# galacticglum/composer

Hardware: AMD Instinct MI355X
Metric: MIDI-event tokens/sec (train, seq=1024) (higher is better)
Workload: dtype bf16; 1 GPU; 6L/8H/d512 Transformer train step, seq=1024, B=128/GPU, dropout 0.10, Adam lr 1e-3, synthetic int32 event ids (vocab 390), random-init weights; global_batch=128, seq_len=1024, parallelism=dp1

## Files before the change

### composer_amd/csrc/attention.hip

```cpp
#include "common.h"

typedef __attribute__((address_space(3))) bf16x4 lds_bf16x4;

__device__ __forceinline__ int rho(int r, int h) { return (r & 3) + 8 * (r >> 2) + 4 * h; }
__device__ __forceinline__ void both_halves(float v, float& a, float& b) {
    uint32_t u = __builtin_bit_cast(uint32_t, v), u2 = u;
    asm volatile("s_nop 1\n\tv_permlane32_swap_b32 %0, %1" : "+v"(u), "+v"(u2));
    const uint32_t r[2] = {u, u2};
    a = __builtin_bit_cast(float, r[0]);
    b = __builtin_bit_cast(float, r[1]);
}
__device__ __forceinline__ float half_max(float v) { float a, b; both_halves(v, a, b); return fmaxf(a, b); }
__device__ __forceinline__ float half_sum(float v) { float a, b; both_halves(v, a, b); return a + b; }

template <typename T> struct AT;
template <> struct AT<bf16_t> {
    static constexpr int KSTEP = 16;
    static constexpr int VN = 8;
    typedef bf16x8 frag;
    static constexpr bool EXACT = false;
};
template <> struct AT<float> {
    static constexpr int KSTEP = 2;
    static constexpr int VN = 4;
    typedef float frag;
    static constexpr bool EXACT = true;
};

template <typename T> using frag_t = typename AT<T>::frag;

template <typename T, int D> struct Occ {
    static constexpr int MINW = (std::is_same<T, float>::value && D == 128) ? 1 : 2;
#ifndef ATTN_MINW_Q
#define ATTN_MINW_Q 3
#endif
    static constexpr int MINW_Q = (std::is_same<T, bf16_t>::value && D <= 64) ? ATTN_MINW_Q : MINW;
};

template <typename T, int D> struct Geo {
    static constexpr int DP = D < 32 ? 32 : D;
    static constexpr int DT = DP / 32;
    static constexpr int S = std::is_same<T, float>::value ? DP + 1 : DP + 8;
    static constexpr int NS = D / AT<T>::KSTEP;
};

template <typename T> __device__ __forceinline__ f32x16 mfma32(frag_t<T> a, frag_t<T> b, f32x16 c);
template <> __device__ __forceinline__ f32x16 mfma32<bf16_t>(bf16x8 a, bf16x8 b, f32x16 c) {
    return __builtin_amdgcn_mfma_f32_32x32x16_bf16(a, b, c, 0, 0, 0);
}
template <> __device__ __forceinline__ f32x16 mfma32<float>(float a, float b, f32x16 c) {
    return __builtin_amdgcn_mfma_f32_32x32x2f32(a, b, c, 0, 0, 0);
}

template <typename T, int D>
__device__ __forceinline__ void stage_rows(T* img, const T* __restrict__ g, int64_t gstride, int row0, int row_end,
                                           int nrows, int tid) {
    constexpr int VN = AT<T>::VN, DP = Geo<T, D>::DP, S = Geo<T, D>::S;
    constexpr int CPR = DP / VN;
    for (int c = tid; c < nrows * CPR; c += 256) {
        int r = c / CPR, cc = c % CPR;
        Vec16<T> v;
#pragma unroll
        for (int j = 0; j < VN; j++) v.set(j, 0.f);
        if (row0 + r < row_end && cc * VN < D) v = ld16(g + (int64_t)(row0 + r) * gstride + cc * VN);
        if (std::is_same<T, float>::value) {
#pragma unroll
            for (int j = 0; j < VN; j++) img[r * S + cc * VN + j] = from_f32<T>(v.get(j));
        } else {
            st16(img + r * S + cc * VN, v);
        }
    }
}

template <typename T, int D, int ROWS = 64> struct Stager {
    static constexpr int VN = AT<T>::VN, DP = Geo<T, D>::DP, S = Geo<T, D>::S;
    static constexpr int CPR = (D < DP ? D : DP) / VN;
    static constexpr int NC = (ROWS * CPR + 255) / 256;
    static constexpr bool WHOLE = (ROWS * CPR) % 256 == 0;
    Vec16<T> r[NC];
    __device__ __forceinline__ void load(const T* __restrict__ g, int64_t gstride, int row0, int row_end, int tid) {
        if constexpr (!std::is_same<T, float>::value || D >= 32) {
            typedef __attribute__((ext_vector_type(4))) uint32_t u32x4;
            const int64_t span = ((int64_t)(row_end - 1) * gstride + D) * (int64_t)sizeof(T);
            const __amdgpu_buffer_rsrc_t rsrc = __builtin_amdgcn_make_buffer_rsrc((void*)g, 0, (int)span, 0x00020000);
#pragma unroll
            for (int i = 0; i < NC; i++) {
                const int c = tid + 256 * i;
                const int row = c / CPR, cc = c % CPR;
                int off = (int)(((int64_t)(row0 + row) * gstride + cc * VN) * (int64_t)sizeof(T));
                if (!WHOLE && c >= ROWS * CPR) off = 0x7FFFFFF0;
                const u32x4 w = __builtin_amdgcn_raw_buffer_load_b128(rsrc, off, 0, 0);
                r[i].v = __builtin_bit_cast(decltype(r[i].v), w);
            }
            return;
        }
#pragma unroll
        for (int i = 0; i < NC; i++) {
            const int c = tid + 256 * i;
            const int row = c / CPR, cc = c % CPR;
#pragma unroll
            for (int j = 0; j < VN; j++) r[i].set(j, 0.f);
            if (c < ROWS * CPR && row0 + row < row_end && cc * VN < D) r[i] = ld16(g + (int64_t)(row0 + row) * gstride + cc * VN);
        }
    }
    __device__ __forceinline__ void store(T* img, int tid) const {
#pragma unroll
        for (int i = 0; i < NC; i++) {
            const int c = tid + 256 * i;
            const int row = c / CPR, cc = c % CPR;
            if (WHOLE || c < ROWS * CPR) {
                if constexpr (std::is_same<T, float>::value) {
#pragma unroll
                    for (int j = 0; j < VN; j++) img[row * S + cc * VN + j] = r[i].get(j);
                } else {
                    st16(img + row * S + cc * VN, r[i]);
                }
            }
        }
    }
};

template <typename T, int D>
__device__ __forceinline__ void load_bfrags(frag_t<T>* f, const T* __restrict__ g,
                                            int64_t gstride, int row, bool valid, int h) {
    constexpr int NS = Geo<T, D>::NS;
#pragma unroll
    for (int s = 0; s < NS; s++) {
        if constexpr (std::is_same<T, float>::value) {
            f[s] = valid ? g[(int64_t)row * gstride + 2 * s + h] : 0.f;
        } else {
            bf16x8 z;
#pragma unroll
            for (int j = 0; j < 8; j++) z[j] = (bf16_t)0.f;
            f[s] = valid ? *reinterpret_cast<const bf16x8*>(g + (int64_t)row * gstride + 16 * s + 8 * h) : z;
        }
    }
}

template <typename T, int D>
__device__ __forceinline__ f32x16 mma_rows(const T* img, int row0, const frag_t<T>* bf,
                                           int lane, f32x16 acc) {
    constexpr int NS = Geo<T, D>::NS, S = Geo<T, D>::S;
    const int r = row0 + (lane & 31), h = lane >> 5;
#pragma unroll
    for (int s = 0; s < NS; s++) {
        frag_t<T> a;
        if constexpr (std::is_same<T, float>::value) a = img[r * S + 2 * s + h];
        else a = *reinterpret_cast<const bf16x8*>(img + r * S + 16 * s + 8 * h);
        acc = mfma32<T>(a, bf[s], acc);
    }
    return acc;
}

template <typename T, int D>
__device__ __forceinline__ f32x16 mma_acc_b(const T* img, int krow0, int dt, const f32x16& x, int lane, f32x16 acc) {
    constexpr int S = Geo<T, D>::S;
    const int h = lane >> 5;
    if constexpr (std::is_same<T, float>::value) {
#pragma unroll
        for (int r = 0; r < 16; r++) {
            float a = img[(krow0 + rho(r, h)) * S + 32 * dt + (lane & 31)];
            acc = __builtin_amdgcn_mfma_f32_32x32x2f32(a, x[r], acc, 0, 0, 0);
        }
    } else {
        const int G = lane >> 4, q = (lane & 15) >> 2, p = lane & 3;
        const int col = 32 * dt + 16 * (G & 1) + 4 * p;
#pragma unroll
        for (int s = 0; s < 2; s++) {
            const int kr = krow0 + 16 * s + 4 * (G >> 1) + q;
            bf16x4 lo = __builtin_amdgcn_ds_read_tr16_b64_v4bf16((lds_bf16x4*)(img + kr * S + col));
            bf16x4 hi = __builtin_amdgcn_ds_read_tr16_b64_v4bf16((lds_bf16x4*)(img + (kr + 8) * S + col));
            bf16x8 a, b;
#pragma unroll
            for (int j = 0; j < 4; j++) {
                a[j] = lo[j];
                a[4 + j] = hi[j];
            }
#pragma unroll
            for (int j = 0; j < 8; j++) b[j] = (bf16_t)x[8 * s + j];
            acc = __builtin_amdgcn_mfma_f32_32x32x16_bf16(a, b, acc, 0, 0, 0);
        }
    }
    return acc;
}

#define LOG2E_F 1.4426950408889634f
__device__ __forceinline__ float fast_exp2(float x) { return __builtin_amdgcn_exp2f(x); }
__device__ __forceinline__ float max3(float a, float b, float c) { return fmaxf(fmaxf(a, b), c); }
__device__ __forceinline__ float max16(const f32x16& s) {
    float a = max3(s[0], s[1], s[2]), b = max3(s[3], s[4], s[5]), c = max3(s[6], s[7], s[8]);
    float d = max3(s[9], s[10], s[11]), e = max3(s[12], s[13], s[14]);
    return max3(max3(a, b, c), max3(d, e, s[15]), a);
}

__device__ __forceinline__ f32x2 exp2_scaled16(f32x16& s, float c, float negm, f32x2 sum) {
    float s0 = sum[0], s1 = sum[1];
#pragma unroll
    for (int r = 0; r < 16; r += 2) {
        const float p0 = fast_exp2(fmaf(s[r], c, negm)), p1 = fast_exp2(fmaf(s[r + 1], c, negm));
        s0 += p0;
        s1 += p1;
        s[r] = p0;
        s[r + 1] = p1;
    }
    return f32x2{s0, s1};
}
__device__ __forceinline__ void pin16(f32x16& v) {
#pragma unroll
    for (int r = 0; r < 16; r++) {
        float x = v[r];
        asm("" : "+v"(x));
        v[r] = x;
    }
}

template <bool PIN = false>
__device__ __forceinline__ void mask16_qlane(f32x16& v, uint32_t rowh, int k0, int h, uint32_t thr) {
    const uint32_t gg = ((uint32_t)(k0 >> 2) + (uint32_t)h) * ATTN_G;
#pragma unroll
    for (int g4 = 0; g4 < 4; g4++) {
        const uint32_t x = rowh ^ (gg + (uint32_t)(2 * g4) * ATTN_G);
        v[4 * g4 + 0] = (__umul24(x, ATTN_C0) >= thr) ? v[4 * g4 + 0] : 0.f;
        v[4 * g4 + 1] = (__umul24(x, ATTN_C1) >= thr) ? v[4 * g4 + 1] : 0.f;
        v[4 * g4 + 2] = (__umul24(x, ATTN_C2) >= thr) ? v[4 * g4 + 2] : 0.f;
        v[4 * g4 + 3] = (__umul24(x, ATTN_C3) >= thr) ? v[4 * g4 + 3] : 0.f;
    }
    if (PIN) pin16(v);
}

template <typename T, int D>
__device__ __forceinline__ void store_t_tile(T* __restrict__ out, int64_t ostride, int row, bool valid, int dt,
                                             const f32x16& y, float mul, int h) {
    if constexpr (std::is_same<T, bf16_t>::value && D % 32 == 0) {
#pragma unroll
        for (int gp = 0; gp < 4; gp += 2) {
            uint32_t w[2][2];
#pragma unroll
            for (int k = 0; k < 2; k++)
#pragma unroll
                for (int j = 0; j < 2; j++) {
                    typedef __attribute__((ext_vector_type(2))) __bf16 bf2;
                    const bf2 t = {(bf16_t)(y[4 * (gp + k) + 2 * j] * mul), (bf16_t)(y[4 * (gp + k) + 2 * j + 1] * mul)};
                    w[k][j] = __builtin_bit_cast(uint32_t, t);
                }
#pragma unroll
            for (int j = 0; j < 2; j++) asm volatile("s_nop 1\n\tv_permlane32_swap_b32 %0, %1" : "+v"(w[0][j]), "+v"(w[1][j]));
            typedef __attribute__((ext_vector_type(4))) uint32_t u32x4;
            const u32x4 v = {w[0][0], w[0][1], w[1][0], w[1][1]};
            if (valid) *reinterpret_cast<u32x4*>(out + (int64_t)row * ostride + 32 * dt + 8 * (gp + h)) = v;
        }
        return;
    }
    if (!valid) return;
#pragma unroll
    for (int g = 0; g < 4; g++) {
        int d = 32 * dt + 8 * g + 4 * h;
        if (d < D) {
            if constexpr (std::is_same<T, float>::value) {
                f32x4 v = {y[4 * g] * mul, y[4 * g + 1] * mul, y[4 * g + 2] * mul, y[4 * g + 3] * mul};
                *reinterpret_cast<f32x4*>(out + (int64_t)row * ostride + d) = v;
            } else {
                bf16x4 v;
#pragma unroll
                for (int j = 0; j < 4; j++) v[j] = (bf16_t)(y[4 * g + j] * mul);
                *reinterpret_cast<bf16x4*>(out + (int64_t)row * ostride + d) = v;
            }
        }
    }
}

template <typename T, int D>
__device__ __forceinline__ void colsum_t_tiles(float* __restrict__ bias_grad, bool valid, const f32x16* y, float mul, int h,
                                               int lane) {
    constexpr int DT = Geo<T, D>::DT;
    const int l = lane & 31;
#pragma unroll
    for (int t0 = 0; t0 < DT; t0 += 2) {
        constexpr int dummy = 0;
        (void)dummy;
        const bool pair = t0 + 1 < DT;
        float v[32];
#pragma unroll
        for (int r = 0; r < 16; r++) {
            v[r] = valid ? y[t0][r] * mul : 0.f;
            v[16 + r] = (pair && valid) ? y[pair ? t0 + 1 : t0][r] * mul : 0.f;
        }
        if (pair) {
#pragma unroll
            for (int k = 0; k < 16; k++) {
                const float keep = (l & 16) ? v[k + 16] : v[k], send = (l & 16) ? v[k] : v[k + 16];
                v[k] = keep + __shfl_xor(send, 16);
            }
        } else {
#pragma unroll
            for (int k = 0; k < 16; k++) v[k] += __shfl_xor(v[k], 16);
        }
#pragma unroll
        for (int s = 8; s >= 1; s >>= 1) {
#pragma unroll
            for (int k = 0; k < s; k++) {
                const float keep = (l & s) ? v[k + s] : v[k], send = (l & s) ? v[k] : v[k + s];
                v[k] = keep + __shfl_xor(send, s);
            }
        }
        const int idx = pair ? l : (l & 15);
        const int d = 32 * (t0 + (idx >> 4)) + 8 * ((idx & 15) >> 2) + 4 * h + (idx & 3);
        if ((pair || l < 16) && d < D) atomicAdd(bias_grad + d, v[0]);
    }
}

__device__ __forceinline__ int pair_block(int ph, int nb, int x) {
    if ((int)gridDim.x == nb && nb > 1) return ph == 0 ? nb - 1 - x : -1;
    const int hi = nb - 1 - x;
    if (ph == 0) return hi;
    return x < hi ? x : -1;
}

__device__ __forceinline__ void xcd_block(int& bx, int& by, int H) {
    const int gx = gridDim.x, gy = gridDim.y;
    if (gy & 7) { bx = blockIdx.x; by = blockIdx.y; return; }
    const int L = blockIdx.x + gx * blockIdx.y;
    const int xcd = L & 7, slot = L >> 3;
    bx = slot % gx;
    by = (slot / gx) * 8 + xcd;
    const int bb = by / H;
    by = bb * H + (by % H + bb) % H;
}

__device__ __forceinline__ void attn_job(int plan_u, int nb, int H, int& by, int& qb0, int& qb1) {
    if (plan_u < 0) {
// ... 532 lines not shown
            const bool more = qts + QT < Tn;
            const int qt0 = qts + wq;
            if (more) {
                sq.load(qg, rs, qts + QT, Tn, tid);
                so.load(dog, E, qts + QT, Tn, tid);
                load_rows(qts + QT);
            }
#pragma unroll
            for (int sub = 0; sub < 2; sub++) {
                const int qb0 = qt0 + 32 * sub;
                if (!INT && (qb0 + 31 < k0w || qb0 >= Tn || k0w >= Tn)) continue;
                f32x16 s, dp;
#pragma unroll
                for (int r = 0; r < 16; r++) { s[r] = 0.f; dp[r] = 0.f; }
                s = mma_rows<T, D>(Qs, 32 * sub, kf, lane, s);
                dp = mma_rows<T, D>(Os, 32 * sub, vf, lane, dp);
                f32x4 lq[4], dq4[4];
                __attribute__((ext_vector_type(4))) uint32_t rh4[4];
#pragma unroll
                for (int g = 0; g < 4; g++) {
                    const int ql = 32 * sub + 8 * g + 4 * h;
                    lq[g] = *reinterpret_cast<const f32x4*>(Ls + ql);
                    dq4[g] = *reinterpret_cast<const f32x4*>(Ls + QT + ql);
                    if constexpr (DROP) rh4[g] = *reinterpret_cast<const __attribute__((ext_vector_type(4))) uint32_t*>(Ls + 2 * QT + ql);
                }
                f32x16 pt;
#pragma unroll
                for (int r = 0; r < 16; r++) {
                    if constexpr (EXACT) pt[r] = expf(s[r] * scale - lq[r >> 2][r & 3]);
                    else pt[r] = fast_exp2(fmaf(s[r], c2, -lq[r >> 2][r & 3]));
                }
                if constexpr (!INT) {
                    const bool edge = EXACT || (qb0 < k0w + 32) || (qb0 + 32 > Tn) || (k0w + 32 > Tn);
                    if (edge) {
#pragma unroll
                        for (int r = 0; r < 16; r++) {
                            const int qq = qt0 + 32 * sub + rho(r, h);
                            if ((key > qq) || (qq >= Tn) || !kvalid) pt[r] = 0.f;
                        }
                    }
                }
#pragma unroll
                for (int r = 0; r < 16; r++) {
                    const float p = pt[r];
                    if constexpr (EXACT || !DROP) {
                        float dpv = dp[r];
                        float pd = p;
                        if constexpr (DROP) {
                            const bool keep = __umul24(rh4[r >> 2][r & 3] ^ kgG, kC) >= drop.thr;
                            dpv = keep ? dpv : 0.f;
                            pd = keep ? p : 0.f;
                        }
                        pt[r] = pd;
                        s[r] = p * (dpv - dq4[r >> 2][r & 3]);
                    } else {
                        const bool keep = __umul24(rh4[r >> 2][r & 3] ^ kgG, kC) >= drop.thr;
                        const float pd = keep ? p : 0.f;
                        pt[r] = pd;
                        s[r] = fmaf(pd, dp[r], -(p * dq4[r >> 2][r & 3]));
                    }
                }
#pragma unroll
                for (int dt = 0; dt < G::DT; dt++) {
                    dv[dt] = mma_acc_b<T, D>(Os, 32 * sub, dt, pt, lane, dv[dt]);
                    dk[dt] = mma_acc_b<T, D>(Qs, 32 * sub, dt, s, lane, dk[dt]);
                }
            }
            if (more) {
                if constexpr (KS) __syncthreads();
                T* nbuf = Qb + (KS ? 0 : (sb ^ 1)) * 2 * IMG;
                sq.store(nbuf, tid);
                so.store(nbuf + IMG, tid);
                store_rows(Lb + (KS ? 0 : (sb ^ 1)) * 3 * QT, qts + QT);
            }
            __syncthreads();
        };
        int qt0 = qstart, it = 0;
        const int diag_end = EXACT ? Tn : min(Tn, KS ? k0w + 32 : qstart + 128);
        for (; qt0 < diag_end; qt0 += QT, it++) tile(std::false_type{}, qt0, it);
        for (; qt0 + QT <= Tn; qt0 += QT, it++) tile(std::true_type{}, qt0, it);
        for (; qt0 < Tn; qt0 += QT, it++) tile(std::false_type{}, qt0, it);
        if constexpr (KS) {
            float* mg = reinterpret_cast<float*>(smem_raw);
            if (wave > 0) {
#pragma unroll
                for (int dt = 0; dt < G::DT; dt++)
#pragma unroll
                    for (int r = 0; r < 16; r++) {
                        mg[(((wave - 1) * 2 * G::DT + 2 * dt) * 16 + r) * 64 + lane] = dk[dt][r];
                        mg[(((wave - 1) * 2 * G::DT + 2 * dt + 1) * 16 + r) * 64 + lane] = dv[dt][r];
                    }
            }
            __syncthreads();
            if (wave > 0) continue;
#pragma unroll
            for (int w = 0; w < 3; w++)
#pragma unroll
                for (int dt = 0; dt < G::DT; dt++)
#pragma unroll
                    for (int r = 0; r < 16; r++) {
                        dk[dt][r] += mg[((w * 2 * G::DT + 2 * dt) * 16 + r) * 64 + lane];
                        dv[dt][r] += mg[((w * 2 * G::DT + 2 * dt + 1) * 16 + r) * 64 + lane];
                    }
        }
        const float row_rs = (lr.rstd && kvalid) ? lr.rstd[(int64_t)b * Tn + key] : 1.f;
#pragma unroll
        for (int dt = 0; dt < G::DT; dt++) {
            store_t_tile<T, D>(dkg, rs, key, kvalid, dt, dk[dt], scale * keep_scale * row_rs, h);
            store_t_tile<T, D>(dvg, rs, key, kvalid, dt, dv[dt], keep_scale * row_rs, h);
        }
        if (bias_grad) {
            colsum_t_tiles<T, D>(bias_grad + E + hd * D, kvalid, dk, scale * keep_scale, h, lane);
            colsum_t_tiles<T, D>(bias_grad + 2 * E + hd * D, kvalid, dv, keep_scale, h, lane);
        }
    }
}
template <typename T, int D, bool DROP>
__global__ __launch_bounds__(256, (Occ<T, D>::MINW)) void attn_dkv_kernel(const T* __restrict__ qkv, const T* __restrict__ d_o,
                                                                          const float* __restrict__ lse,
                                                                          const float* __restrict__ delta, T* __restrict__ dqkv,
                                                                          float* __restrict__ bias_grad, int Tn, int H, float scale,
                                                                          DropCfg drop) {
    attn_dkv_body<T, D, DROP, 0>(qkv, d_o, lse, delta, dqkv, bias_grad, Tn, H, scale, drop, nullptr, 0);
}
template <typename T, int D, bool DROP>
__global__ __launch_bounds__(256, (Occ<T, D>::MINW)) void attn_dkv_ln_kernel(const T* __restrict__ qkv, const T* __restrict__ d_o,
                                                                          const float* __restrict__ lse,
                                                                          const float* __restrict__ delta, T* __restrict__ dqkv,
                                                                          float* __restrict__ bias_grad, int Tn, int H, float scale,
                                                                          DropCfg drop, AttnLnRows lr) {
    attn_dkv_body<T, D, DROP, 0>(qkv, d_o, lse, delta, dqkv, bias_grad, Tn, H, scale, drop, nullptr, 0, lr);
}
template <typename T, int D, bool DROP>
__global__ __launch_bounds__(256, 2) void attn_bwd_ks_kernel(const T* __restrict__ qkv, const T* __restrict__ o, const T* __restrict__ d_o,
                                                             const float* __restrict__ lse, float* __restrict__ delta, T* __restrict__ dqkv,
                                                             float* __restrict__ bias_grad, int Tn, int H, float scale, DropCfg drop) {
    const int x = blockIdx.x, nqb = (int)gridDim.x >> 1;
    if (x & 1) attn_dq_body<T, D, DROP, 1>(qkv, o, d_o, lse, delta, dqkv, bias_grad, Tn, H, scale, drop, -1, nqb - 1 - (x >> 1));
    else attn_dkv_body<T, D, DROP, 2>(qkv, d_o, lse, delta, dqkv, bias_grad, Tn, H, scale, drop, o, x >> 1);
}
template <typename T, int D, bool DROP>
__global__ __launch_bounds__(256, 2) void attn_dq_ks_kernel(const T* __restrict__ qkv, const T* __restrict__ o, const T* __restrict__ d_o,
                                                            const float* __restrict__ lse, float* __restrict__ delta, T* __restrict__ dqkv,
                                                            float* __restrict__ bias_grad, int Tn, int H, float scale, DropCfg drop) {
    attn_dq_body<T, D, DROP, 1>(qkv, o, d_o, lse, delta, dqkv, bias_grad, Tn, H, scale, drop, -1, (int)gridDim.x - 1 - (int)blockIdx.x);
}
template <typename T, int D, bool DROP>
__global__ __launch_bounds__(256, 2) void attn_dkv_ks_kernel(const T* __restrict__ qkv, const T* __restrict__ d_o, const float* __restrict__ lse,
                                                             const float* __restrict__ delta, T* __restrict__ dqkv, float* __restrict__ bias_grad,
                                                             int Tn, int H, float scale, DropCfg drop) {
    attn_dkv_body<T, D, DROP, 1>(qkv, d_o, lse, delta, dqkv, bias_grad, Tn, H, scale, drop, nullptr, (int)blockIdx.x);
}

int colsum_run(void* stream, const void* X, int ldx, float* out, int rows, int cols, int dtype, float* det_ws, size_t det_ws_bytes);
static int attn_grid_x(int Tn, int BH) {
    const int nb = cdiv(Tn, 128), pairs = (nb + 1) / 2;
    return (nb > 1 && (int64_t)pairs * BH < 512) ? nb : pairs;
}
static int attn_plan_u(int Tn, int BH, int wgs_per_cu) {
    const int nb = cdiv(Tn, 128), pairs = (nb + 1) / 2;
    if (nb < 2 || (BH & 7) || (int64_t)pairs * BH < 512 || wgs_per_cu < 1) return -1;
    const int rows_x = BH / 8, slots = 32 * wgs_per_cu;
    const int rounds = rows_x * pairs / slots;
    const int paired_rows = rounds > 0 ? rounds * slots / pairs : rows_x / 4;
    const int u = rows_x - paired_rows;
    return u > 0 ? u : -1;
}
static dim3 attn_plan_grid(int Tn, int BH, int u) {
    if (u < 0) return dim3(attn_grid_x(Tn, BH), BH);
    const int nb = cdiv(Tn, 128), pairs = (nb + 1) / 2, rows_x = BH / 8;
    return dim3(8 * ((rows_x - u) * pairs + u * nb), 1);
}
static bool attn_key_split(int Tn, int BH, int D, bool bf16) {
    if (!bf16 || D > 32 || Tn < 64) return false;
    static const int mode = [] { const char* e = getenv("COMPOSER_ATTN_KS"); return e ? atoi(e) : -1; }();
    if (mode == 0) return false;
    if (mode == 1) return true;
    return (int64_t)cdiv(Tn, 128) * BH <= 128;
}
template <typename K> static int attn_wgs_per_cu(K kernel, size_t smem) {
    int n = 0;
    if (hipOccupancyMaxActiveBlocksPerMultiprocessor(&n, kernel, 256, smem) != hipSuccess) { (void)hipGetLastError(); return 0; }
    return n;
}
template <typename T, int D> static size_t attn_ks_smem() { return 4 * 256 * Geo<T, D>::S * sizeof(T); }
template <typename T, int D> static bool attn_ks_available() {
    static const bool ok = [] {
        const int ks = (int)attn_ks_smem<T, D>(), kv = ks / 2 + 3 * 256 * (int)sizeof(float);
        const void* big[] = {(const void*)attn_fwd_kernel<T, D, true, false, true>, (const void*)attn_fwd_kernel<T, D, false, false, true>,
                             (const void*)attn_bwd_ks_kernel<T, D, true>, (const void*)attn_bwd_ks_kernel<T, D, false>,
                             (const void*)attn_dq_ks_kernel<T, D, true>, (const void*)attn_dq_ks_kernel<T, D, false>};
        const void* half[] = {(const void*)attn_dkv_ks_kernel<T, D, true>, (const void*)attn_dkv_ks_kernel<T, D, false>};
        bool good = true;
        for (const void* f : big) good = good && hipFuncSetAttribute(f, hipFuncAttributeMaxDynamicSharedMemorySize, ks) == hipSuccess;
        for (const void* f : half) good = good && hipFuncSetAttribute(f, hipFuncAttributeMaxDynamicSharedMemorySize, kv) == hipSuccess;
        if (!good) (void)hipGetLastError();
        return good;
    }();
    return ok;
}
template <typename T, int D>
static int launch_fwd(hipStream_t s, const void* qkv, void* o, float* lse, int B, int Tn, int H, float scale, DropCfg d,
                      const float* amask) {
    if constexpr (std::is_same<T, bf16_t>::value && D <= 32) {
        const size_t smem_ks = attn_ks_smem<T, D>();
        if (!amask && attn_ks_available<T, D>() && attn_key_split(Tn, B * H, D, true)) {
            const dim3 grid(cdiv(Tn, 32), B * H);
            PROF_START(3, s);
            if (d.thr) attn_fwd_kernel<T, D, true, false, true><<<grid, 256, smem_ks, s>>>((const T*)qkv, (T*)o, lse, Tn, H, scale, d, -1, nullptr);
            else attn_fwd_kernel<T, D, false, false, true><<<grid, 256, smem_ks, s>>>((const T*)qkv, (T*)o, lse, Tn, H, scale, d, -1, nullptr);
            PROF_STOP(3, s, 2.0 * B * H * (double)Tn * Tn * D, (double)B * Tn * H * (4.0 * D * sizeof(T) + 4.0));
            KERNEL_CHECK();
            return CMP_OK;
        }
    }
    size_t smem = 4 * 64 * Geo<T, D>::S * sizeof(T);
    if (smem > 65536) {
        HIP_CHECK(hipFuncSetAttribute((const void*)attn_fwd_kernel<T, D, true>, hipFuncAttributeMaxDynamicSharedMemorySize, (int)smem));
        HIP_CHECK(hipFuncSetAttribute((const void*)attn_fwd_kernel<T, D, false>, hipFuncAttributeMaxDynamicSharedMemorySize, (int)smem));
    }
    static const int wgs_per_cu = attn_wgs_per_cu(attn_fwd_kernel<T, D, true>, smem);
    const int plan_u = attn_plan_u(Tn, B * H, wgs_per_cu);
    const dim3 grid = attn_plan_grid(Tn, B * H, plan_u);
    const double flops = 2.0 * B * H * (double)Tn * Tn * D;
    if (amask) {
        if (smem > 65536) {
            HIP_CHECK(hipFuncSetAttribute((const void*)attn_fwd_kernel<T, D, true, true>, hipFuncAttributeMaxDynamicSharedMemorySize, (int)smem));
            HIP_CHECK(hipFuncSetAttribute((const void*)attn_fwd_kernel<T, D, false, true>, hipFuncAttributeMaxDynamicSharedMemorySize, (int)smem));
        }
        if (d.thr) attn_fwd_kernel<T, D, true, true><<<grid, 256, smem, s>>>((const T*)qkv, (T*)o, lse, Tn, H, scale, d, plan_u, amask);
        else attn_fwd_kernel<T, D, false, true><<<grid, 256, smem, s>>>((const T*)qkv, (T*)o, lse, Tn, H, scale, d, plan_u, amask);
        KERNEL_CHECK();
        return CMP_OK;
    }
    PROF_START(3, s);
    if (d.thr) attn_fwd_kernel<T, D, true><<<grid, 256, smem, s>>>((const T*)qkv, (T*)o, lse, Tn, H, scale, d, plan_u, nullptr);
    else attn_fwd_kernel<T, D, false><<<grid, 256, smem, s>>>((const T*)qkv, (T*)o, lse, Tn, H, scale, d, plan_u, nullptr);
    PROF_STOP(3, s, flops, (double)B * Tn * H * (4.0 * D * sizeof(T) + 4.0));
    KERNEL_CHECK();
    return CMP_OK;
}
template <typename T, int D>
static int launch_bwd(hipStream_t s, const void* qkv, const void* o, const void* d_o, const float* lse, float* delta,
                      void* dqkv, int B, int Tn, int H, float scale, DropCfg d, float* bias_grad, AttnLnRows lr) {
    if constexpr (std::is_same<T, bf16_t>::value) {
        if (lr.rstd) {
            size_t smem = 4 * 64 * Geo<T, D>::S * sizeof(T);
            if (smem + 1536 > 65536) {
                HIP_CHECK(hipFuncSetAttribute((const void*)attn_dq_ln_kernel<T, D, true>, hipFuncAttributeMaxDynamicSharedMemorySize, (int)smem));
                HIP_CHECK(hipFuncSetAttribute((const void*)attn_dq_ln_kernel<T, D, false>, hipFuncAttributeMaxDynamicSharedMemorySize, (int)smem));
                HIP_CHECK(hipFuncSetAttribute((const void*)attn_dkv_ln_kernel<T, D, true>, hipFuncAttributeMaxDynamicSharedMemorySize, (int)smem + 1536));
                HIP_CHECK(hipFuncSetAttribute((const void*)attn_dkv_ln_kernel<T, D, false>, hipFuncAttributeMaxDynamicSharedMemorySize, (int)smem + 1536));
            }
            const double fl = (double)B * H * (double)Tn * Tn * D;
            static const int wgs_per_cu_ln = attn_wgs_per_cu(attn_dq_ln_kernel<T, D, true>, smem);
            const int plan_u = attn_plan_u(Tn, B * H, wgs_per_cu_ln);
            const dim3 qgrid = attn_plan_grid(Tn, B * H, plan_u);
            const dim3 kgrid(attn_grid_x(Tn, B * H), B * H);
            PROF_START(4, s);
            if (d.thr) attn_dq_ln_kernel<T, D, true><<<qgrid, 256, smem, s>>>((const T*)qkv, (const T*)o, (const T*)d_o, lse, delta, (T*)dqkv, bias_grad, Tn, H, scale, d, plan_u, lr);
            else attn_dq_ln_kernel<T, D, false><<<qgrid, 256, smem, s>>>((const T*)qkv, (const T*)o, (const T*)d_o, lse, delta, (T*)dqkv, bias_grad, Tn, H, scale, d, plan_u, lr);
            PROF_STOP(4, s, 3.0 * fl, (double)B * Tn * H * (6.0 * D * sizeof(T) + 8.0));
            KERNEL_CHECK();
            PROF_START(5, s);
            if (d.thr) attn_dkv_ln_kernel<T, D, true><<<kgrid, 256, smem + 384 * sizeof(float), s>>>((const T*)qkv, (const T*)d_o, lse, delta, (T*)dqkv, bias_grad, Tn, H, scale, d, lr);
            else attn_dkv_ln_kernel<T, D, false><<<kgrid, 256, smem + 384 * sizeof(float), s>>>((const T*)qkv, (const T*)d_o, lse, delta, (T*)dqkv, bias_grad, Tn, H, scale, d, lr);
            PROF_STOP(5, s, 4.0 * fl, (double)B * Tn * H * (6.0 * D * sizeof(T) + 8.0));
            KERNEL_CHECK();
            return CMP_OK;
        }
    } else {
        CMP_REQUIRE(!lr.rstd, "attention backward: LayerNorm row scaling exists in bf16 only");
    }
    if constexpr (std::is_same<T, bf16_t>::value && D <= 32) {
        const size_t smem_ks = attn_ks_smem<T, D>(), smem_kv = smem_ks / 2 + 3 * 256 * sizeof(float);
        if (attn_ks_available<T, D>() && attn_key_split(Tn, B * H, D, true)) {
            const double flk = (double)B * H * (double)Tn * Tn * D;
            float* const bias_out = bias_grad;
            bias_grad = nullptr;
            auto bias_pass = [&]() -> int {
                return bias_out ? colsum_run(s, dqkv, 3 * H * D, bias_out, B * Tn, 3 * H * D, CMP_BF16, nullptr, 0) : CMP_OK;
            };
            if ((int64_t)2 * cdiv(Tn, 32) * B * H > 512) {
                const dim3 g1(cdiv(Tn, 32), B * H);
                PROF_START(4, s);
                if (d.thr) attn_dq_ks_kernel<T, D, true><<<g1, 256, smem_ks, s>>>((const T*)qkv, (const T*)o, (const T*)d_o, lse, delta, (T*)dqkv, bias_grad, Tn, H, scale, d);
                else attn_dq_ks_kernel<T, D, false><<<g1, 256, smem_ks, s>>>((const T*)qkv, (const T*)o, (const T*)d_o, lse, delta, (T*)dqkv, bias_grad, Tn, H, scale, d);
                PROF_STOP(4, s, 3.0 * flk, (double)B * Tn * H * (6.0 * D * sizeof(T) + 8.0));
                KERNEL_CHECK();
                PROF_START(5, s);
                if (d.thr) attn_dkv_ks_kernel<T, D, true><<<g1, 256, smem_kv, s>>>((const T*)qkv, (const T*)d_o, lse, delta, (T*)dqkv, bias_grad, Tn, H, scale, d);
                else attn_dkv_ks_kernel<T, D, false><<<g1, 256, smem_kv, s>>>((const T*)qkv, (const T*)d_o, lse, delta, (T*)dqkv, bias_grad, Tn, H, scale, d);
                PROF_STOP(5, s, 4.0 * flk, (double)B * Tn * H * (6.0 * D * sizeof(T) + 8.0));
                KERNEL_CHECK();
                return bias_pass();
            }
            const dim3 kgrid(2 * cdiv(Tn, 32), B * H);
            PROF_START(5, s);
            if (d.thr) attn_bwd_ks_kernel<T, D, true><<<kgrid, 256, smem_ks, s>>>((const T*)qkv, (const T*)o, (const T*)d_o, lse, delta, (T*)dqkv, bias_grad, Tn, H, scale, d);
            else attn_bwd_ks_kernel<T, D, false><<<kgrid, 256, smem_ks, s>>>((const T*)qkv, (const T*)o, (const T*)d_o, lse, delta, (T*)dqkv, bias_grad, Tn, H, scale, d);
            PROF_STOP(5, s, 7.0 * flk, (double)B * Tn * H * (9.0 * D * sizeof(T) + 8.0));
            KERNEL_CHECK();
            return bias_pass();
        }
    }
    dim3 grid(attn_grid_x(Tn, B * H), B * H);
    static const int bias_pass_mib = [] { const char* e = getenv("COMPOSER_ATTN_BIAS_PASS"); return e ? atoi(e) : 16; }();
    float* bias_out = nullptr;
    if (bias_grad && std::is_same<T, bf16_t>::value && (int64_t)B * Tn * 3 * H * D * 2 <= (int64_t)bias_pass_mib << 20) { bias_out = bias_grad; bias_grad = nullptr; }
    size_t smem = 4 * 64 * Geo<T, D>::S * sizeof(T);
    if (smem + 1536 > 65536) {
        HIP_CHECK(hipFuncSetAttribute((const void*)attn_dq_kernel<T, D, true>, hipFuncAttributeMaxDynamicSharedMemorySize, (int)smem));
        HIP_CHECK(hipFuncSetAttribute((const void*)attn_dq_kernel<T, D, false>, hipFuncAttributeMaxDynamicSharedMemorySize, (int)smem));
        HIP_CHECK(hipFuncSetAttribute((const void*)attn_dkv_kernel<T, D, true>, hipFuncAttributeMaxDynamicSharedMemorySize, (int)smem + 1536));
        HIP_CHECK(hipFuncSetAttribute((const void*)attn_dkv_kernel<T, D, false>, hipFuncAttributeMaxDynamicSharedMemorySize, (int)smem + 1536));
    }
    const double fl = (double)B * H * (double)Tn * Tn * D;
    PROF_START(4, s);
    static const int wgs_per_cu = attn_wgs_per_cu(attn_dq_kernel<T, D, true>, smem);
    const int plan_u = attn_plan_u(Tn, B * H, wgs_per_cu);
    const dim3 qgrid = attn_plan_grid(Tn, B * H, plan_u);
    if (d.thr) attn_dq_kernel<T, D, true><<<qgrid, 256, smem, s>>>((const T*)qkv, (const T*)o, (const T*)d_o, lse, delta, (T*)dqkv, bias_grad, Tn, H, scale, d, plan_u);
    else attn_dq_kernel<T, D, false><<<qgrid, 256, smem, s>>>((const T*)qkv, (const T*)o, (const T*)d_o, lse, delta, (T*)dqkv, bias_grad, Tn, H, scale, d, plan_u);
    PROF_STOP(4, s, 3.0 * fl, (double)B * Tn * H * (6.0 * D * sizeof(T) + 8.0));
    KERNEL_CHECK();
    PROF_START(5, s);
    if (d.thr) attn_dkv_kernel<T, D, true><<<grid, 256, smem + 384 * sizeof(float), s>>>((const T*)qkv, (const T*)d_o, lse, delta, (T*)dqkv, bias_grad, Tn, H, scale, d);
    else attn_dkv_kernel<T, D, false><<<grid, 256, smem + 384 * sizeof(float), s>>>((const T*)qkv, (const T*)d_o, lse, delta, (T*)dqkv, bias_grad, Tn, H, scale, d);
    PROF_STOP(5, s, 4.0 * fl, (double)B * Tn * H * (6.0 * D * sizeof(T) + 8.0));
    KERNEL_CHECK();
    if (bias_out) return colsum_run(s, dqkv, 3 * H * D, bias_out, B * Tn, 3 * H * D, CMP_BF16, nullptr, 0);
    return CMP_OK;
}

#define DISPATCH_D(T, fn, ...)                                                         \
    switch (D) {                                                                       \
        case 16: return fn<T, 16>(__VA_ARGS__);                                        \
        case 32: return fn<T, 32>(__VA_ARGS__);                                        \
        case 64: return fn<T, 64>(__VA_ARGS__);                                        \
        case 128: return fn<T, 128>(__VA_ARGS__);                                      \
        default: cmp_set_error("attention: head size %d unsupported (16/32/64/128)", D); \
                 return CMP_ERR_INVALID;                                               \
    }

extern "C" int cmp_k_attn_fwd(void* stream, const void* qkv, void* o, float* lse, int B, int T, int H, int D, int scale,
                              int dtype, float p_drop, uint64_t seed, uint32_t rng_stream) {
    return attn_fwd_run(stream, qkv, o, lse, B, T, H, D, scale ? 1.0f / sqrtf((float)D) : 1.0f, dtype, p_drop, seed, rng_stream, nullptr);
}

int attn_fwd_run(void* stream, const void* qkv, void* o, float* lse, int B, int T, int H, int D, float sc, int dtype, float p_drop,
                 uint64_t seed, uint32_t rng_stream, const float* amask) {
    if (B * T == 0) return CMP_OK;
    hipStream_t s = (hipStream_t)stream;
    DropCfg d = make_drop(p_drop, seed, rng_stream);
    if (dtype == CMP_BF16) { DISPATCH_D(bf16_t, launch_fwd, s, qkv, o, lse, B, T, H, sc, d, amask) }
    else { DISPATCH_D(float, launch_fwd, s, qkv, o, lse, B, T, H, sc, d, amask) }
}

template <typename T>
__global__ __launch_bounds__(256) void attn_probs_kernel(const T* __restrict__ qkv, const float* __restrict__ lse,
                                                         const float* __restrict__ amask, float* __restrict__ out, int q0, int Tn,
                                                         int H, int D, float scale, DropCfg drop) {
    const int bh = blockIdx.y, i = q0 + blockIdx.x, b = bh / H, hd = bh % H;
    const int E = H * D;
    const int64_t rs = 3 * E;
    const T* qrow = qkv + ((int64_t)b * Tn + i) * rs + hd * D;
    const float l = lse[(int64_t)bh * Tn + i];
    const uint32_t rowh = attn_row_hash(drop.seed, drop.stream, (uint32_t)(bh * Tn + i));
    float* orow = out + ((int64_t)bh * (Tn - q0) + (i - q0)) * Tn;
    for (int j = threadIdx.x; j < Tn; j += blockDim.x) {
        const T* krow = qkv + ((int64_t)b * Tn + j) * rs + E + hd * D;
        float sdot = 0.f;
        for (int d = 0; d < D; d++) sdot = fmaf(to_f32<T>(qrow[d]), to_f32<T>(krow[d]), sdot);
        float v = sdot * scale;
        if (j > i) v = -1e4f;
        if (amask) v += amask[(int64_t)b * Tn + j];
        float pr = expf(v - l);
        if (drop.thr) pr = attn_elem_hash(rowh, (uint32_t)j) >= drop.thr ? pr * drop.scale : 0.f;
        orow[j] = pr;
    }
}

int attn_probs_run(void* stream, const void* qkv, const float* lse, const float* amask, float* out, int B, int q0, int T, int H, int D,
                   float sc, int dtype, float p_drop, uint64_t seed, uint32_t rng_stream) {
    if (B * (T - q0) <= 0) return CMP_OK;
    hipStream_t s = (hipStream_t)stream;
    const DropCfg d = make_drop(p_drop, seed, rng_stream);
    const dim3 grid(T - q0, B * H);
    if (dtype == CMP_BF16) attn_probs_kernel<bf16_t><<<grid, 256, 0, s>>>((const bf16_t*)qkv, lse, amask, out, q0, T, H, D, sc, d);
    else attn_probs_kernel<float><<<grid, 256, 0, s>>>((const float*)qkv, lse, amask, out, q0, T, H, D, sc, d);
    KERNEL_CHECK();
    return CMP_OK;
}

static thread_local float* t_attn_bias_next = nullptr;
extern "C" int cmp_attn_bwd_bias_next(float* out) {
    t_attn_bias_next = out;
    return CMP_OK;
}

static thread_local AttnLnRows t_attn_ln_next;
extern "C" int cmp_attn_bwd_ln_next(const float* rstd) {
    t_attn_ln_next = AttnLnRows{rstd};
    return CMP_OK;
}

extern "C" int cmp_k_attn_bwd(void* stream, const void* qkv, const void* o, const void* d_o, const float* lse,
                              float* delta_ws, void* dqkv, int B, int T, int H, int D, int scale, int dtype,
                              float p_drop, uint64_t seed, uint32_t rng_stream) {
    float* bias_grad = t_attn_bias_next;
    t_attn_bias_next = nullptr;
    const AttnLnRows lr = t_attn_ln_next;
    t_attn_ln_next = AttnLnRows();
    return attn_bwd_run(stream, qkv, o, d_o, lse, delta_ws, dqkv, B, T, H, D, scale ? 1.0f / sqrtf((float)D) : 1.0f, dtype, p_drop, seed,
                        rng_stream, bias_grad, lr);
}

int attn_bwd_run(void* stream, const void* qkv, const void* o, const void* d_o, const float* lse, float* delta_ws, void* dqkv,
                 int B, int T, int H, int D, float sc, int dtype, float p_drop, uint64_t seed, uint32_t rng_stream,
                 float* bias_grad, AttnLnRows lr) {
    if (B * T == 0) return CMP_OK;
    hipStream_t s = (hipStream_t)stream;
    DropCfg d = make_drop(p_drop, seed, rng_stream);
    if (dtype == CMP_BF16) { DISPATCH_D(bf16_t, launch_bwd, s, qkv, o, d_o, lse, delta_ws, dqkv, B, T, H, sc, d, bias_grad, lr) }
    else { DISPATCH_D(float, launch_bwd, s, qkv, o, d_o, lse, delta_ws, dqkv, B, T, H, sc, d, bias_grad, lr) }
}
```

Baseline: 4.918 million tokens/s.

## Add fused single-kernel attention backward for bf16 D=64 with dQ slab combine

Adds a 512-thread attention backward kernel that keeps a 512-key block of K in LDS. It computes dK/dV in registers and dQ through an LDS dS image, fusing the delta computation and the separate dq/dkv passes into one sweep over query tiles. dQ for query rows beyond the first key block is written as partial fp32 slabs and summed by a small combine kernel. This costs extra slab memory traffic and a second launch, but avoids recomputing the scores and probabilities twice. It is enabled by default when Tn>512 and the block count is large enough, and it also records which backward path ran.

```diff
diff --git a/composer_amd/csrc/attention.hip b/composer_amd/csrc/attention.hip
--- a/composer_amd/csrc/attention.hip
+++ b/composer_amd/csrc/attention.hip
@@ -1,4 +1,5 @@
 #include "common.h"
+#include <mutex>
 
 typedef __attribute__((address_space(3))) bf16x4 lds_bf16x4;
 
@@ -72,11 +73,11 @@
     }
 }
 
-template <typename T, int D, int ROWS = 64> struct Stager {
+template <typename T, int D, int ROWS = 64, int NT = 256> struct Stager {
     static constexpr int VN = AT<T>::VN, DP = Geo<T, D>::DP, S = Geo<T, D>::S;
     static constexpr int CPR = (D < DP ? D : DP) / VN;
-    static constexpr int NC = (ROWS * CPR + 255) / 256;
-    static constexpr bool WHOLE = (ROWS * CPR) % 256 == 0;
+    static constexpr int NC = (ROWS * CPR + NT - 1) / NT;
+    static constexpr bool WHOLE = (ROWS * CPR) % NT == 0;
     Vec16<T> r[NC];
     __device__ __forceinline__ void load(const T* __restrict__ g, int64_t gstride, int row0, int row_end, int tid) {
         if constexpr (!std::is_same<T, float>::value || D >= 32) {
@@ -85,7 +86,7 @@
             const __amdgpu_buffer_rsrc_t rsrc = __builtin_amdgcn_make_buffer_rsrc((void*)g, 0, (int)span, 0x00020000);
 #pragma unroll
             for (int i = 0; i < NC; i++) {
-                const int c = tid + 256 * i;
+                const int c = tid + NT * i;
                 const int row = c / CPR, cc = c % CPR;
                 int off = (int)(((int64_t)(row0 + row) * gstride + cc * VN) * (int64_t)sizeof(T));
                 if (!WHOLE && c >= ROWS * CPR) off = 0x7FFFFFF0;
@@ -96,7 +97,7 @@
         }
 #pragma unroll
         for (int i = 0; i < NC; i++) {
-            const int c = tid + 256 * i;
+            const int c = tid + NT * i;
             const int row = c / CPR, cc = c % CPR;
 #pragma unroll
             for (int j = 0; j < VN; j++) r[i].set(j, 0.f);
@@ -106,7 +107,7 @@
     __device__ __forceinline__ void store(T* img, int tid) const {
 #pragma unroll
         for (int i = 0; i < NC; i++) {
-            const int c = tid + 256 * i;
+            const int c = tid + NT * i;
             const int row = c / CPR, cc = c % CPR;
             if (WHOLE || c < ROWS * CPR) {
                 if constexpr (std::is_same<T, float>::value) {
@@ -152,6 +153,22 @@
     return acc;
 }
 
+template <int S>
+__device__ __forceinline__ bf16x8 tr_afrag(const bf16_t* img, int krow0, int col0, int lane) {
+    const int G = lane >> 4, q = (lane & 15) >> 2, p = lane & 3;
+    const int col = col0 + 16 * (G & 1) + 4 * p;
+    const int kr = krow0 + 4 * (G >> 1) + q;
+    const bf16x4 lo = __builtin_amdgcn_ds_read_tr16_b64_v4bf16((lds_bf16x4*)(img + kr * S + col));
+    const bf16x4 hi = __builtin_amdgcn_ds_read_tr16_b64_v4bf16((lds_bf16x4*)(img + (kr + 8) * S + col));
+    bf16x8 a;
+#pragma unroll
+    for (int j = 0; j < 4; j++) {
+        a[j] = lo[j];
+        a[4 + j] = hi[j];
+    }
+    return a;
+}
+
 template <typename T, int D>
 __device__ __forceinline__ f32x16 mma_acc_b(const T* img, int krow0, int dt, const f32x16& x, int lane, f32x16 acc) {
     constexpr int S = Geo<T, D>::S;
@@ -163,19 +180,10 @@
             acc = __builtin_amdgcn_mfma_f32_32x32x2f32(a, x[r], acc, 0, 0, 0);
         }
     } else {
-        const int G = lane >> 4, q = (lane & 15) >> 2, p = lane & 3;
-        const int col = 32 * dt + 16 * (G & 1) + 4 * p;
 #pragma unroll
         for (int s = 0; s < 2; s++) {
-            const int kr = krow0 + 16 * s + 4 * (G >> 1) + q;
-            bf16x4 lo = __builtin_amdgcn_ds_read_tr16_b64_v4bf16((lds_bf16x4*)(img + kr * S + col));
-            bf16x4 hi = __builtin_amdgcn_ds_read_tr16_b64_v4bf16((lds_bf16x4*)(img + (kr + 8) * S + col));
-            bf16x8 a, b;
-#pragma unroll
-            for (int j = 0; j < 4; j++) {
-                a[j] = lo[j];
-                a[4 + j] = hi[j];
-            }
+            const bf16x8 a = tr_afrag<S>(img, krow0 + 16 * s, 32 * dt, lane);
+            bf16x8 b;
 #pragma unroll
             for (int j = 0; j < 8; j++) b[j] = (bf16_t)x[8 * s + j];
             acc = __builtin_amdgcn_mfma_f32_32x32x16_bf16(a, b, acc, 0, 0, 0);
@@ -1014,6 +1022,269 @@
     attn_dkv_body<T, D, DROP, 1>(qkv, d_o, lse, delta, dqkv, bias_grad, Tn, H, scale, drop, nullptr, (int)blockIdx.x);
 }
 
+#define FB_KEYS 512
+#define FB_DSS (FB_KEYS + 8)
+static constexpr size_t attn_fb_smem() {
+    return (size_t)(FB_KEYS * 72 + 64 * FB_DSS + 2 * 64 * 72) * sizeof(bf16_t) + 3 * 64 * sizeof(float);
+}
+template <bool DROP>
+__global__ __launch_bounds__(512, 2) void attn_bwd_fused_kernel(const bf16_t* __restrict__ qkv, const bf16_t* __restrict__ o,
+                                                               const bf16_t* __restrict__ d_o, const float* __restrict__ lse,
+                                                               float* __restrict__ delta, bf16_t* __restrict__ dqkv,
+                                                               float* __restrict__ dq_slab, float* __restrict__ bias_grad, int Tn,
+                                                               int H, int BH, float scale, DropCfg drop) {
+    typedef bf16_t T;
+    constexpr int D = 64;
+    using G = Geo<T, D>;
+    constexpr int S = G::S, QT = 64;
+    static_assert(S == 72 && G::NS == 4 && G::DT == 2, "layout");
+    extern __shared__ __attribute__((aligned(16))) char smem_raw[];
+    T* Kimg = reinterpret_cast<T*>(smem_raw);
+    T* dSimg = Kimg + FB_KEYS * S;
+    T* Qs = dSimg + 64 * FB_DSS;
+    T* Os = Qs + 64 * S;
+    float* Lb = reinterpret_cast<float*>(Os + 64 * S);
+    const int tid = threadIdx.x, lane = tid & 63, h = lane >> 5;
+    const int wave = __builtin_amdgcn_readfirstlane(tid >> 6);
+    const int kb = (int)blockIdx.x / BH, by = (int)blockIdx.x % BH;
+    const int b = by / H, hd = by % H;
+    const int E = H * D;
+    const int64_t rs = 3 * E;
+    const T* qg = qkv + (int64_t)b * Tn * rs + hd * D;
+    const T* kg = qg + E;
+    const T* vg = qg + 2 * E;
+    const T* dog = d_o + (int64_t)b * Tn * E + hd * D;
+    const T* ogl = o + (int64_t)b * Tn * E + hd * D;
+    T* dqg = dqkv + (int64_t)b * Tn * rs + hd * D;
+    T* dkg = dqg + E;
+    T* dvg = dqg + 2 * E;
+    const float c2 = scale * LOG2E_F;
+    const float keep_scale = DROP ? drop.scale : 1.0f;
+    const int kbase = kb * FB_KEYS;
+    const int kend = min(FB_KEYS, Tn - kbase);
+
+    for (int c = tid; c < FB_KEYS * 8; c += 512) {
+        const int r = c >> 3, cc = c & 7;
+        Vec16<T> v;
+#pragma unroll
+        for (int j = 0; j < 8; j++) v.set(j, 0.f);
+        if (r < kend) v = ld16(kg + (int64_t)(kbase + r) * rs + cc * 8);
+        st16(Kimg + r * S + cc * 8, v);
+    }
+    int k0[2], key[2];
+    bool kvalid[2];
+    uint32_t kgG[2], kC[2];
+    frag_t<T> vf[2][G::NS];
+#pragma unroll
+    for (int j = 0; j < 2; j++) {
+        k0[j] = kbase + 32 * (wave + 8 * j);
+        key[j] = k0[j] + (lane & 31);
+        kvalid[j] = key[j] < Tn;
+        load_bfrags<T, D>(vf[j], vg, rs, key[j], kvalid[j], h);
+        kgG[j] = ((uint32_t)key[j] >> 2) * ATTN_G;
+        const int k3 = key[j] & 3;
+        kC[j] = k3 == 0 ? ATTN_C0 : (k3 == 1 ? ATTN_C1 : (k3 == 2 ? ATTN_C2 : ATTN_C3));
+    }
+    f32x16 dk[2][G::DT], dv[2][G::DT];
+#pragma unroll
+    for (int j = 0; j < 2; j++)
+#pragma unroll
+        for (int dt = 0; dt < G::DT; dt++)
+#pragma unroll
+            for (int r = 0; r < 16; r++) { dk[j][dt][r] = 0.f; dv[j][dt][r] = 0.f; }
+
+    Stager<T, D, QT, 512> sq, so, sO;
+    float st_l = 0.f;
+    auto load_tile = [&](int qt) {
+        sq.load(qg, rs, qt, Tn, tid);
+        so.load(dog, E, qt, Tn, tid);
+        sO.load(ogl, E, qt, Tn, tid);
+        st_l = lse[(int64_t)by * Tn + min(qt + (tid >> 3), Tn - 1)];
+    };
+    auto store_tile = [&](int qt) {
+        sq.store(Qs, tid);
+        so.store(Os, tid);
+        float dsum = 0.f;
+#pragma unroll
+        for (int j = 0; j < 8; j++) dsum = fmaf(sO.r[0].get(j), so.r[0].get(j), dsum);
+        dsum += __shfl_xor(dsum, 1);
+        dsum += __shfl_xor(dsum, 2);
+        dsum += __shfl_xor(dsum, 4);
+        if ((tid & 7) == 0) {
+            const int row = tid >> 3, q = qt + row;
+            Lb[row] = st_l * LOG2E_F;
+            Lb[64 + row] = dsum / keep_scale;
+            reinterpret_cast<uint32_t*>(Lb)[128 + row] = attn_row_hash(drop.seed, drop.stream, (uint32_t)(by * Tn + q));
+            if (kb == 0 && q < Tn) delta[(int64_t)by * Tn + q] = dsum;
+        }
+    };
+    const int qstart = kbase;
+    load_tile(qstart);
+    store_tile(qstart);
+    __syncthreads();
+
+    auto tile = [&](auto interior, const int qt) __attribute__((always_inline)) {
+        constexpr bool INT = decltype(interior)::value;
+        const bool more = qt + QT < Tn;
+        if (more) load_tile(qt + QT);
+#pragma unroll
+        for (int j = 0; j < 2; j++) {
+            const int kl0 = 32 * (wave + 8 * j);
+            frag_t<T> kf[G::NS];
+#pragma unroll
+            for (int s = 0; s < G::NS; s++) kf[s] = *reinterpret_cast<const bf16x8*>(Kimg + (kl0 + (lane & 31)) * S + 16 * s + 8 * h);
+#pragma unroll
+            for (int qs = 0; qs < 2; qs++) {
+                const int q0 = qt + 32 * qs;
+                T* dsw = dSimg + (32 * qs) * FB_DSS + kl0 + (lane & 31);
+                if (!INT && (q0 + 31 < k0[j] || q0 >= Tn || k0[j] >= Tn)) {
+#pragma unroll
+                    for (int r = 0; r < 16; r++) dsw[rho(r, h) * FB_DSS] = (T)0.f;
+                    continue;
+                }
+                f32x16 s, dp;
+#pragma unroll
+                for (int r = 0; r < 16; r++) { s[r] = 0.f; dp[r] = 0.f; }
+                s = mma_rows<T, D>(Qs, 32 * qs, kf, lane, s);
+                dp = mma_rows<T, D>(Os, 32 * qs, vf[j], lane, dp);
+                f32x4 lq[4], dq4[4];
+                __attribute__((ext_vector_type(4))) uint32_t rh4[4];
+#pragma unroll
+                for (int g = 0; g < 4; g++) {
+                    const int ql = 32 * qs + 8 * g + 4 * h;
+                    lq[g] = *reinterpret_cast<const f32x4*>(Lb + ql);
+                    dq4[g] = *reinterpret_cast<const f32x4*>(Lb + 64 + ql);
+                    if constexpr (DROP) rh4[g] = *reinterpret_cast<const __attribute__((ext_vector_type(4))) uint32_t*>(Lb + 128 + ql);
+                }
+                f32x16 pt;
+#pragma unroll
+                for (int r = 0; r < 16; r++) pt[r] = fast_exp2(fmaf(s[r], c2, -lq[r >> 2][r & 3]));
+                if constexpr (!INT) {
+                    const bool edge = (q0 < k0[j] + 32) || (q0 + 32 > Tn) || (k0[j] + 32 > Tn);
+                    if (edge) {
+#pragma unroll
+                        for (int r = 0; r < 16; r++) {
+                            const int qq = q0 + rho(r, h);
+                            if ((key[j] > qq) || (qq >= Tn) || !kvalid[j]) pt[r] = 0.f;
+                        }
+                    }
+                }
+#pragma unroll
+                for (int r = 0; r < 16; r++) {
+                    const float p = pt[r];
+                    if constexpr (!DROP) {
+                        s[r] = p * (dp[r] - dq4[r >> 2][r & 3]);
+                    } else {
+                        const bool keep = __umul24(rh4[r >> 2][r & 3] ^ kgG[j], kC[j]) >= drop.thr;
+                        const float pd = keep ? p : 0.f;
+                        pt[r] = pd;
+                        s[r] = fmaf(pd, dp[r], -(p * dq4[r >> 2][r & 3]));
+                    }
+                }
+#pragma unroll
+                for (int r = 0; r < 16; r++) dsw[rho(r, h) * FB_DSS] = (T)s[r];
+#pragma unroll
+                for (int dt = 0; dt < G::DT; dt++) {
+                    dv[j][dt] = mma_acc_b<T, D>(Os, 32 * qs, dt, pt, lane, dv[j][dt]);
+                    dk[j][dt] = mma_acc_b<T, D>(Qs, 32 * qs, dt, s, lane, dk[j][dt]);
+                }
+            }
+        }
+        __syncthreads();
+        if (more) store_tile(qt + QT);
+        if (wave < 4) {
+            const int dt = wave & 1, qs = wave >> 1;
+            const int nk = min(min((kend + 31) & ~31, qt + QT - kbase), FB_KEYS);
+            f32x16 acc;
+#pragma unroll
+            for (int r = 0; r < 16; r++) acc[r] = 0.f;
+            const T* dsr = dSimg + (32 * qs + (lane & 31)) * FB_DSS + 4 * h;
+            for (int kk = 0; kk < nk; kk += 32) {
+#pragma unroll
+                for (int s = 0; s < 2; s++) {
+                    const bf16x8 a = tr_afrag<S>(Kimg, kk + 16 * s, 32 * dt, lane);
+                    const bf16x4 lo = *reinterpret_cast<const bf16x4*>(dsr + kk + 16 * s);
+                    const bf16x4 hi = *reinterpret_cast<const bf16x4*>(dsr + kk + 16 * s + 8);
+                    bf16x8 bb;
+#pragma unroll
+                    for (int jj = 0; jj < 4; jj++) {
+                        bb[jj] = lo[jj];
+                        bb[4 + jj] = hi[jj];
+                    }
+                    acc = __builtin_amdgcn_mfma_f32_32x32x16_bf16(a, bb, acc, 0, 0, 0);
+                }
+            }
+            const int q = qt + 32 * qs + (lane & 31);
+            const bool qvalid = q < Tn;
+            if (qt < FB_KEYS) {
+                store_t_tile<T, D>(dqg, rs, q, qvalid, dt, acc, scale * keep_scale, h);
+                if (bias_grad) colsum_t_tiles<T, 32>(bias_grad + hd * D + 32 * dt, qvalid, &acc, scale * keep_scale, h, lane);
+            } else if (qvalid) {
+                float* dst = dq_slab + (((int64_t)kb * BH + by) * (Tn - FB_KEYS) + (q - FB_KEYS)) * D + 32 * dt + 4 * h;
+#pragma unroll
+                for (int g = 0; g < 4; g++) *reinterpret_cast<f32x4*>(dst + 8 * g) = f32x4{acc[4 * g], acc[4 * g + 1], acc[4 * g + 2], acc[4 * g + 3]};
+            }
+        }
+        __syncthreads();
+    };
+    int qt = qstart;
+    const int diag_end = min(Tn, qstart + FB_KEYS);
+    for (; qt < diag_end; qt += QT) tile(std::false_type{}, qt);
+    for (; qt + QT <= Tn; qt += QT) tile(std::true_type{}, qt);
+    for (; qt < Tn; qt += QT) tile(std::false_type{}, qt);
+
+#pragma unroll
+    for (int j = 0; j < 2; j++) {
+#pragma unroll
+        for (int dt = 0; dt < G::DT; dt++) {
+            store_t_tile<T, D>(dkg, rs, key[j], kvalid[j], dt, dk[j][dt], scale * keep_scale, h);
+            store_t_tile<T, D>(dvg, rs, key[j], kvalid[j], dt, dv[j][dt], keep_scale, h);
+        }
+        if (bias_grad) {
+            colsum_t_tiles<T, D>(bias_grad + E + hd * D, kvalid[j], dk[j], scale * keep_scale, h, lane);
+            colsum_t_tiles<T, D>(bias_grad + 2 * E + hd * D, kvalid[j], dv[j], keep_scale, h, lane);
+        }
+    }
+}
+
+__global__ __launch_bounds__(256) void attn_dq_combine_kernel(const float* __restrict__ dq_slab, bf16_t* __restrict__ dqkv,
+                                                              float* __restrict__ bias_grad, int Tn, int H, int BH, float mul) {
+    constexpr int D = 64;
+    __shared__ float red[32][D + 1];
+    const int by = blockIdx.y, b = by / H, hd = by % H;
+    const int row = threadIdx.x >> 3, c = threadIdx.x & 7;
+    const int q = FB_KEYS + 32 * (int)blockIdx.x + row;
+    float acc[8];
+#pragma unroll
+    for (int j = 0; j < 8; j++) acc[j] = 0.f;
+    if (q < Tn) {
+        const int nkb = q / FB_KEYS + 1;
+        const int64_t rows = Tn - FB_KEYS;
+        for (int kb = 0; kb < nkb; kb++) {
+            const f32x4* p = reinterpret_cast<const f32x4*>(dq_slab + (((int64_t)kb * BH + by) * rows + (q - FB_KEYS)) * D + 8 * c);
+            const f32x4 x = p[0], y = p[1];
+#pragma unroll
+            for (int j = 0; j < 4; j++) {
+                acc[j] += x[j];
+                acc[4 + j] += y[j];
+            }
+        }
+        Vec16<bf16_t> v;
+#pragma unroll
+        for (int j = 0; j < 8; j++) v.set(j, acc[j] * mul);
+        st16(dqkv + ((int64_t)b * Tn + q) * 3 * H * D + hd * D + 8 * c, v);
+    }
+    if (!bias_grad) return;
+#pragma unroll
+    for (int j = 0; j < 8; j++) red[row][8 * c + j] = q < Tn ? acc[j] * mul : 0.f;
+    __syncthreads();
+    if (threadIdx.x < D) {
+        float sum = 0.f;
+        for (int r = 0; r < 32; r++) sum += red[r][threadIdx.x];
+        atomicAdd(bias_grad + hd * D + threadIdx.x, sum);
+    }
+}
+
 int colsum_run(void* stream, const void* X, int ldx, float* out, int rows, int cols, int dtype, float* det_ws, size_t det_ws_bytes);
 static int attn_grid_x(int Tn, int BH) {
     const int nb = cdiv(Tn, 128), pairs = (nb + 1) / 2;
@@ -1102,6 +1373,55 @@
     KERNEL_CHECK();
     return CMP_OK;
 }
+static thread_local int t_attn_bwd_path = 0;
+static bool attn_fused_bwd(int Tn, int BH) {
+    static const int mode = [] { const char* e = getenv("COMPOSER_ATTN_FUSED_BWD"); return e ? atoi(e) : -1; }();
+    if (Tn <= FB_KEYS || mode == 0) return false;
+    if (mode == 1) return true;
+    return (int64_t)cdiv(Tn, FB_KEYS) * BH >= 1024;
+}
+static int attn_fb_slab(size_t bytes, float** out) {
+    static std::mutex mu;
+    static float* buf[64] = {};
+    static size_t cap[64] = {};
+    int dev = 0;
+    HIP_CHECK(hipGetDevice(&dev));
+    CMP_REQUIRE(dev >= 0 && dev < 64, "attention backward: device index %d out of range", dev);
+    std::lock_guard<std::mutex> g(mu);
+    if (cap[dev] < bytes) {
+        void* q = nullptr;
+        HIP_CHECK(hipMalloc(&q, bytes));
+        buf[dev] = (float*)q;
+        cap[dev] = bytes;
+    }
+    *out = buf[dev];
+    return CMP_OK;
+}
+static int launch_bwd_fused(hipStream_t s, const bf16_t* qkv, const bf16_t* o, const bf16_t* d_o, const float* lse, float* delta,
+                            bf16_t* dqkv, int B, int Tn, int H, float scale, DropCfg d, float* bias_grad) {
+    constexpr int D = 64;
+    const int BH = B * H, nkb = cdiv(Tn, FB_KEYS);
+    const size_t smem = attn_fb_smem();
+    static const bool attr_ok = [smem] {
+        return hipFuncSetAttribute((const void*)attn_bwd_fused_kernel<true>, hipFuncAttributeMaxDynamicSharedMemorySize, (int)smem) == hipSuccess &&
+               hipFuncSetAttribute((const void*)attn_bwd_fused_kernel<false>, hipFuncAttributeMaxDynamicSharedMemorySize, (int)smem) == hipSuccess;
+    }();
+    CMP_REQUIRE(attr_ok, "attention backward: the fused kernel's %zu bytes of LDS were refused", smem);
+    float* slab = nullptr;
+    if (const int rc = attn_fb_slab((size_t)nkb * BH * (Tn - FB_KEYS) * D * sizeof(float), &slab)) return rc;
+    double slab_rows = 0;
+    for (int kb = 0; kb < nkb; kb++) slab_rows += Tn - std::max(FB_KEYS, kb * FB_KEYS);
+    const double fl = (double)BH * (double)Tn * Tn * D;
+    PROF_START(5, s);
+    if (d.thr) attn_bwd_fused_kernel<true><<<nkb * BH, 512, smem, s>>>(qkv, o, d_o, lse, delta, dqkv, slab, bias_grad, Tn, H, BH, scale, d);
+    else attn_bwd_fused_kernel<false><<<nkb * BH, 512, smem, s>>>(qkv, o, d_o, lse, delta, dqkv, slab, bias_grad, Tn, H, BH, scale, d);
+    KERNEL_CHECK();
+    attn_dq_combine_kernel<<<dim3(cdiv(Tn - FB_KEYS, 32), BH), 256, 0, s>>>(slab, dqkv, bias_grad, Tn, H, BH, scale * d.scale);
+    PROF_STOP(5, s, 5.0 * fl, (double)B * Tn * H * (8.0 * D * sizeof(bf16_t) + 8.0) + 2.0 * slab_rows * BH * D * sizeof(float));
+    KERNEL_CHECK();
+    t_attn_bwd_path = 2;
+    return CMP_OK;
+}
 template <typename T, int D>
 static int launch_bwd(hipStream_t s, const void* qkv, const void* o, const void* d_o, const float* lse, float* delta,
                       void* dqkv, int B, int Tn, int H, float scale, DropCfg d, float* bias_grad, AttnLnRows lr) {
@@ -1129,6 +1449,7 @@
             else attn_dkv_ln_kernel<T, D, false><<<kgrid, 256, smem + 384 * sizeof(float), s>>>((const T*)qkv, (const T*)d_o, lse, delta, (T*)dqkv, bias_grad, Tn, H, scale, d, lr);
             PROF_STOP(5, s, 4.0 * fl, (double)B * Tn * H * (6.0 * D * sizeof(T) + 8.0));
             KERNEL_CHECK();
+            t_attn_bwd_path = 4;
             return CMP_OK;
         }
     } else {
@@ -1155,6 +1476,7 @@
                 else attn_dkv_ks_kernel<T, D, false><<<g1, 256, smem_kv, s>>>((const T*)qkv, (const T*)d_o, lse, delta, (T*)dqkv, bias_grad, Tn, H, scale, d);
                 PROF_STOP(5, s, 4.0 * flk, (double)B * Tn * H * (6.0 * D * sizeof(T) + 8.0));
                 KERNEL_CHECK();
+                t_attn_bwd_path = 3;
                 return bias_pass();
             }
             const dim3 kgrid(2 * cdiv(Tn, 32), B * H);
@@ -1163,8 +1485,13 @@
             else attn_bwd_ks_kernel<T, D, false><<<kgrid, 256, smem_ks, s>>>((const T*)qkv, (const T*)o, (const T*)d_o, lse, delta, (T*)dqkv, bias_grad, Tn, H, scale, d);
             PROF_STOP(5, s, 7.0 * flk, (double)B * Tn * H * (9.0 * D * sizeof(T) + 8.0));
             KERNEL_CHECK();
+            t_attn_bwd_path = 3;
             return bias_pass();
         }
+    }
+    if constexpr (std::is_same<T, bf16_t>::value && D == 64) {
+        if (attn_fused_bwd(Tn, B * H))
+            return launch_bwd_fused(s, (const T*)qkv, (const T*)o, (const T*)d_o, lse, delta, (T*)dqkv, B, Tn, H, scale, d, bias_grad);
     }
     dim3 grid(attn_grid_x(Tn, B * H), B * H);
     static const int bias_pass_mib = [] { const char* e = getenv("COMPOSER_ATTN_BIAS_PASS"); return e ? atoi(e) : 16; }();
@@ -1191,6 +1518,7 @@
     else attn_dkv_kernel<T, D, false><<<grid, 256, smem + 384 * sizeof(float), s>>>((const T*)qkv, (const T*)d_o, lse, delta, (T*)dqkv, bias_grad, Tn, H, scale, d);
     PROF_STOP(5, s, 4.0 * fl, (double)B * Tn * H * (6.0 * D * sizeof(T) + 8.0));
     KERNEL_CHECK();
+    t_attn_bwd_path = 1;
     if (bias_out) return colsum_run(s, dqkv, 3 * H * D, bias_out, B * Tn, 3 * H * D, CMP_BF16, nullptr, 0);
     return CMP_OK;
 }
@@ -1261,6 +1589,8 @@
     return CMP_OK;
 }
 
+extern "C" int cmp_attn_bwd_last_path(void) { return t_attn_bwd_path; }
+
 static thread_local AttnLnRows t_attn_ln_next;
 extern "C" int cmp_attn_bwd_ln_next(const float* rstd) {
     t_attn_ln_next = AttnLnRows{rstd};
```

New measurement: 3.207 million tokens/s, median of 2. -34.8%, worse.
